# nicochunger/evidence

Hardware: AMD Instinct MI355X
Metric: live_point_logL_evals_per_sec (higher is better)
Workload: dtype f64

## Files before the change

### evidence_amd/csrc/rvll_math.h

```cpp
#pragma once
#include <hip/hip_runtime.h>
#include <stdint.h>

#define RVLL_HD __host__ __device__ __forceinline__

namespace rvll {

RVLL_HD double as_double(uint64_t u) { return __builtin_bit_cast(double, u); }
RVLL_HD uint64_t as_u64(double d) { return __builtin_bit_cast(uint64_t, d); }

struct SincosConsts {
    double S1, S2, S3, S4, S5, S6, C1, C2, C3, C4, C5, C6, TWO_OVER_PI, PIO2_HI, PIO2_LO, MAGIC;
};
RVLL_HD SincosConsts sincos_consts()
{
    return SincosConsts{-1.66666666666666324348e-01, 8.33333333332248946124e-03, -1.98412698298579493134e-04,
                        2.75573137070700676789e-06, -2.50507602534068634195e-08, 1.58969099521155010221e-10,
                        4.16666666666666019037e-02, -1.38888888888741095749e-03, 2.48015872894767294178e-05,
                        -2.75573143513906633035e-07, 2.08757232129817482790e-09, -1.13596475577881948265e-11,
                        6.36619772367581382433e-01, 1.57079632679489655800e+00, 6.12323399573676603587e-17,
                        6755399441055744.0};
}
#if defined(__HIP_DEVICE_COMPILE__)
__device__ __forceinline__ SincosConsts sincos_consts_pinned()
// ... 421 lines not shown
    reduce_dd(x, r, q);
    double sr, cr;
#ifdef RVLL_CR_SERIES_ONLY
    sincos_dd_kernel(r, sr, cr);
#else
    if (__builtin_expect(!sincos_dd_table(r, sr, cr), 0)) sincos_dd_kernel(r, sr, cr);
#endif
    const double s = (q & 1u) ? cr : sr, c = (q & 1u) ? sr : cr;
    const double ss = (q & 2u) ? -s : s, cc = ((q + 1u) & 2u) ? -c : c;
    s_out = x < 0. ? -ss : ss;
    c_out = cc;
}

RVLL_HD double recip_refined(double d)
{
#if defined(__HIP_DEVICE_COMPILE__)
    double y = __builtin_amdgcn_rcp(d);
    double e = __builtin_fma(-d, y, 1.0);
    y = __builtin_fma(y, e, y);
    e = __builtin_fma(-d, y, 1.0);
    return __builtin_fma(y, e, y);
#else
    return 1.0 / d;
#endif
}
RVLL_HD double div_1nr(double n, double d)
{
#if defined(__HIP_DEVICE_COMPILE__)
    double y = __builtin_amdgcn_rcp(d);
    y = __builtin_fma(y, __builtin_fma(-d, y, 1.0), y);
    const double q = n * y;
    return __builtin_fma(__builtin_fma(-d, q, n), y, q);
#else
    return n / d;
#endif
}
RVLL_HD double div_exact(double n, double d) { return div_1nr(n, d); }
RVLL_HD double div_fast(double n, double d) { return div_1nr(n, d); }

RVLL_HD double log_pos(double v)
{
#if defined(__HIP_DEVICE_COMPILE__)
    if (!(v > 0.0 && v < __builtin_inf())) return log(v);
    double m = __builtin_amdgcn_frexp_mant(v);
    int    k = __builtin_amdgcn_frexp_exp(v);
    const bool lowhalf = m < 7.07106781186547524401e-01;
    m = lowhalf ? m + m : m;
    k = lowhalf ? k - 1 : k;
    const double f = m - 1.0;
    const double s = div_fast(f, 2.0 + f);
    const double z = s * s;
    constexpr double L7 = 1.479819860511658591e-01, L6 = 1.531383769920937332e-01, L5 = 1.818357216161805012e-01,
                     L4 = 2.222219843214978396e-01, L3 = 2.857142874366239149e-01, L2 = 3.999999999940941908e-01,
                     L1 = 6.666666666666735130e-01;
    double R;
    asm("v_fma_f64 %0, %1, %2, %3\n\t"
        "v_fma_f64 %0, %1, %0, %4\n\t"
        "v_fma_f64 %0, %1, %0, %5\n\t"
        "v_fma_f64 %0, %1, %0, %6\n\t"
        "v_fma_f64 %0, %1, %0, %7\n\t"
        "v_fma_f64 %0, %1, %0, %8\n\t"
        "v_mul_f64 %0, %0, %1"
        : "=&v"(R)
        : "v"(z), "v"(L7), "v"(L6), "v"(L5), "v"(L4), "v"(L3), "v"(L2), "v"(L1));
    const double hfsq = 0.5 * f * f;
    const double dk = (double)k;
    const double inner = __builtin_fma(s, hfsq + R, dk * 1.90821492927058770002e-10);
    return __builtin_fma(dk, 6.93147180369123816490e-01, -((hfsq - inner) - f));
#else
    return __builtin_log(v);
#endif
}

RVLL_HD void rotate_small(double h, double& s, double& c)
{
    const double h2 = h * h;
    const double sh = h * __builtin_fma(h2, -1.66666666666666666667e-01, 1.0);
    const double ch1 = h2 * __builtin_fma(h2, 4.16666666666666666667e-02, -0.5);
    const double s0 = s, c0 = c;
    s = s0 + __builtin_fma(s0, ch1, c0 * sh);
    c = c0 + __builtin_fma(c0, ch1, -(s0 * sh));
}

RVLL_HD void rotate_mid(double h, double& s, double& c, const SincosConsts& k)
{
    const double S1 = k.S1, S2 = k.S2, S3 = k.S3, S4 = k.S4, S5 = k.S5, S6 = k.S6;
    const double C1 = k.C1, C2 = k.C2, C3 = k.C3, C4 = k.C4, C5 = k.C5, C6 = k.C6;
    double sh, cm1;
#if defined(__HIP_DEVICE_COMPILE__)
    double z, t;
    asm("v_mul_f64 %2, %4, %4\n\t"
        "v_fma_f64 %0, %2, %10, %9\n\t"
        "v_fma_f64 %1, %2, %16, %15\n\t"
        "v_fma_f64 %0, %2, %0, %8\n\t"
        "v_fma_f64 %1, %2, %1, %14\n\t"
        "v_fma_f64 %0, %2, %0, %7\n\t"
        "v_fma_f64 %1, %2, %1, %13\n\t"
        "v_fma_f64 %0, %2, %0, %6\n\t"
        "v_fma_f64 %1, %2, %1, %12\n\t"
        "v_fma_f64 %0, %2, %0, %5\n\t"
        "v_fma_f64 %1, %2, %1, %11\n\t"
        "v_mul_f64 %3, %4, %2\n\t"
        "v_fma_f64 %1, %2, %1, -0.5\n\t"
        "v_fma_f64 %0, %3, %0, %4\n\t"
        "v_mul_f64 %1, %2, %1"
        : "=&v"(sh), "=&v"(cm1), "=&v"(z), "=&v"(t)
        : "v"(h), "s"(S1), "s"(S2), "s"(S3), "s"(S4), "s"(S5), "v"(S6),
          "s"(C1), "s"(C2), "s"(C3), "s"(C4), "s"(C5), "v"(C6));
#else
    const double z = h * h;
    double ps = __builtin_fma(z, S6, S5);
    double pc = __builtin_fma(z, C6, C5);
    ps = __builtin_fma(z, ps, S4);
    pc = __builtin_fma(z, pc, C4);
    ps = __builtin_fma(z, ps, S3);
    pc = __builtin_fma(z, pc, C3);
    ps = __builtin_fma(z, ps, S2);
    pc = __builtin_fma(z, pc, C2);
    ps = __builtin_fma(z, ps, S1);
    pc = __builtin_fma(z, pc, C1);
    const double t = h * z;
    pc = __builtin_fma(z, pc, -0.5);
    sh = __builtin_fma(t, ps, h);
    cm1 = z * pc;
#endif
    const double s0 = s, c0 = c;
    s = __builtin_fma(c0, sh, __builtin_fma(s0, cm1, s0));
    c = __builtin_fma(-s0, sh, __builtin_fma(c0, cm1, c0));
}

RVLL_HD void rotate_mid(double h, double& s, double& c) { rotate_mid(h, s, c, sincos_consts()); }

constexpr double kRotateMidMax = 7.85398163397448279e-01;

template <bool CHECKED>
RVLL_HD void newton_next_sincos(double E, double h, int k, double& s, double& c, const SincosConsts& kc)
{
    if (k == 0) {
        if constexpr (CHECKED) sincos_any(E, s, c, kc);
        else                   sincos_f64(E, s, c, kc);
    } else {
        rotate_mid(h, s, c, kc);
        if (__builtin_expect(!(__builtin_fabs(h) <= kRotateMidMax), 0)) {
            if constexpr (CHECKED) sincos_any(E, s, c, kc);
            else                   sincos_f64(E, s, c, kc);
        }
    }
}

RVLL_HD void quadrant_f32(float sr, float cr, uint32_t uq, float& s_out, float& c_out)
{
    const uint32_t m = 0u - (uq & 1u);
    const uint32_t sb = __builtin_bit_cast(uint32_t, sr), cb = __builtin_bit_cast(uint32_t, cr);
    uint32_t rs, rc;
#if defined(__HIP_DEVICE_COMPILE__)
    asm("v_bfi_b32 %0, %2, %4, %3\n\t"
        "v_bfi_b32 %1, %2, %3, %4"
        : "=&v"(rs), "=&v"(rc) : "v"(m), "v"(sb), "v"(cb));
#else
    rs = (cb & m) | (sb & ~m);
    rc = (sb & m) | (cb & ~m);
#endif
    rs ^= (uq & 2u) << 30;
    rc ^= ((uq + 1u) & 2u) << 30;
    s_out = __builtin_bit_cast(float, rs);
    c_out = __builtin_bit_cast(float, rc);
// ... 94 lines not shown
```

### evidence_amd/csrc/rvll_tile.h

```cpp
#pragma once
#include "rvll_kernels.h"
#include "rvll_math.h"
#include "rvll_special.h"

namespace rvll {

namespace {

constexpr double kTwoPi = 6.283185307179586476925286766559;

__device__ __forceinline__ double slot_get(const rvll_slot s, const double* th)
{
    return s.idx >= 0 ? th[s.idx] : s.val;
}

__device__ __forceinline__ double slot_lds(const rvll_slot* s, const double* th)
{
    const int idx = s->idx;
    const double v = s->val;
    const double tv = th[idx >= 0 ? idx : 0];
    return idx >= 0 ? tv : v;
}

__device__ __forceinline__ double wave_sum(double v)
// ... 123 lines not shown
    const rvll_prior& pr = priors[d];
    const double q = cube_row[d];
    switch (pr.kind) {
    case RVLL_PRIOR_UNIFORM:
        return pr.args[0] + (pr.args[1] - pr.args[0]) * q;
    case RVLL_PRIOR_JEFFREYS:
        return pr.args[0] * pow(pr.args[1] / pr.args[0], q);
    case RVLL_PRIOR_MODJEFFREYS:
        return pr.args[0] * pow(1 + pr.args[1] / pr.args[0], q) - pr.args[0];
    case RVLL_PRIOR_UNIFORMFREQUENCY:
        return pr.args[0] / (1 - q * (pr.args[1] - pr.args[0]) / pr.args[1]);
    case RVLL_PRIOR_NORMAL:
        return (q >= 0. && q <= 1.) ? ndtri_cephes(q) * pr.args[1] + pr.args[0] : NAN;
    case RVLL_PRIOR_LOGNORMAL:
        return (q >= 0. && q <= 1.) ? exp(pr.args[0] * ndtri_cephes(q)) * pr.args[2] + pr.args[1] : NAN;
    case RVLL_PRIOR_TRUNCRAYLEIGH: {
        const double sg = pr.args[0], xm = pr.args[1];
        const double A = 1 - exp(-(xm * xm) / (2 * (sg * sg)));
        return sqrt(-2 * (sg * sg) * log(1 - (q * A))); }
    case RVLL_PRIOR_TABLE:
        return table_ppf(pr, q);
    case RVLL_PRIOR_ALPHA:
        return alpha_ppf(q, pr.args[0], pr.args[1]);
    case RVLL_PRIOR_SORTED_UNIFORM:
    case RVLL_PRIOR_SORTED_LOGUNIFORM:
        return sorted_prior(priors, D, cube_row, d, pr.kind);
    default:
        return NAN;
    }
}

__device__ double prior_heavy(const rvll_prior& pr, double q)
{
    const bool direct = pr.table_post != 0;
    if (pr.kind == RVLL_PRIOR_BETA)
        return beta_ppf_table(q, pr.args[0], pr.args[1], pr.args[2], pr.table_cdf, pr.table_x, direct);
    return gamma_ppf_table(q, pr.args[0], pr.args[1], pr.args[2], pr.table_cdf, pr.table_x, direct);
}

__device__ __forceinline__ double prior_heavy_slim(const rvll_prior& pr, double q, double umax, bool& deferred)
{
    if (pr.table_post != 0 && q > 0. && q < 1.) {
        const double ud = logit_fast(q);
        if (fabs(ud) <= umax) {
            const double z = quintic_table(pr.table_cdf, pr.table_x, ud);
            return pr.kind == RVLL_PRIOR_BETA ? 1. / (1. + exp(-z)) : exp(z) * (1.0 / pr.args[1]);
        }
    }
    deferred = true;
    return NAN;
}

__device__ __forceinline__ double walk_normal(unsigned long long seed, unsigned long long ctr)
{
    const double u1 = uniform01(seed, ctr), u2 = uniform01(seed, ctr + 1);
    double sn, cs;
    sincos_f64(kTwoPi * u2, sn, cs);
    return sqrt(-2. * log_pos(1. - u1)) * cs;
}

struct ItemCtx {
    const double* pp;
    const double* ins;
    const double* dr;
    const double* lin;
    int* nfail;
    int* anyfail;
    int* jfail;
    const int* wide;
    int* pflags;
};

__device__ __forceinline__ bool f32_astray(float E, float Mf, float tolf) { return !(fabsf(E - Mf) <= 1.0f + tolf); }

template <int PREC, bool FAILCHECK, bool EXTRAS = true, bool CR = false, int NP = 0>
__device__ __forceinline__ double eval_item(const LoglikeArgs& a, const ItemCtx& cx, int pl, int j)
{
    const double t  = a.t[j];
    const double y  = a.y[j];
    const double s2 = a.s2[j];
    const int    in = a.inst[j];

    const double2 oj = *reinterpret_cast<const double2*>(cx.ins + (pl * a.Ni + in) * 2);
    double rvm = 0. + oj.x;
    const double var = s2 + oj.y;

    const int Np = NP > 0 ? NP : a.Np;
    if (Np > 0) {
        const bool wide = __builtin_amdgcn_readfirstlane(*cx.wide) != 0;
        bool point_failed = false;
        if constexpr (FAILCHECK) point_failed = cx.anyfail[pl] != 0;
        double ksum = 0.;
#pragma clang loop unroll_count(NP > 0 ? NP : 1)
        for (int ip = 0; ip < Np; ++ip) {
            const double* P = cx.pp + (pl * Np + ip) * kPlanetFields;
            const double2 p01 = *reinterpret_cast<const double2*>(P);
            const double2 p23 = *reinterpret_cast<const double2*>(P + 2);
            const double2 p45 = *reinterpret_cast<const double2*>(P + 4);
            const double  C0  = P[6];
            const double ec = p23.y;
            double rv;
            if (FAILCHECK && point_failed && j >= cx.jfail[pl * Np + ip]) {
                rv = p45.x + C0;
            } else if constexpr (PREC == RVLL_PREC_FP64) {
                const double M = p01.x * (t - p01.y) + p23.x;
                double E = M, s, c, dE = __builtin_inf();
#ifdef RVLL_LOCAL_CONSTS
                const SincosConsts kc = sincos_consts_pinned();
#else
                const SincosConsts kc = sincos_consts();
#endif
                const bool shortcut = a.itmax > kSafeSteps && !wide;
                if (shortcut) {
                    int steps = 0;
                    do {
                        newton_next_sincos<false>(E, dE, steps, s, c, kc);
                        const double f  = E - ec * s - M;
                        const double fp = 1 - ec * c;
                        const double En = E - div_exact(f, fp);
                        dE = En - E;
                        E = En;
                        ++steps;
                    } while (fabs(dE) > a.tol && steps < kSafeSteps);
                }
                if constexpr (CR) {
                    if (!shortcut && a.itmax > kSafeSteps) {
                        int steps = 0;
                        do {
                            newton_next_sincos<true>(E, dE, steps, s, c, kc);
                            const double f  = E - ec * s - M;
                            const double fp = 1 - ec * c;
                            const double En = E - div_exact(f, fp);
                            dE = En - E;
                            E = En;
                            ++steps;
                        } while (fabs(dE) > a.tol && steps < kSafeSteps);
                    }
                }
                bool hit_itmax = false, wander = false;
                if (__builtin_expect(!(fabs(dE) <= a.tol), 0)) {
#ifdef RVLL_AB_PRIO
                    __builtin_amdgcn_s_setprio(2);
#endif
                    int steps = shortcut ? kSafeSteps : 0;
                    if constexpr (CR) { E = M; steps = 0; }
                    do {
#ifdef RVLL_CR_FAKE
                        sincos_any(E, s, c, kc);
#else
                        if constexpr (CR)            sincos_cr(E, s, c);
                        else if (steps < kSafeSteps) newton_next_sincos<true>(E, dE, steps, s, c, kc);
                        else                         sincos_any(E, s, c, kc);
#endif
                        const double f  = E - ec * s - M;
                        const double fp = 1 - ec * c;
                        const double En = E - div_exact(f, fp);
                        dE = En - E;
                        E = En;
                        ++steps;
                    } while (fabs(dE) > a.tol && steps < a.itmax);
                    hit_itmax = steps >= a.itmax;
                    if (steps > kSafeSteps) {
                        atomicOr(&cx.pflags[pl], RVLL_FLAG_WANDERED);
                        if constexpr (!CR) { if (a.cr_redo) { atomicOr(cx.nfail, 2); wander = true; } }
                    }
#ifdef RVLL_AB_PRIO
                    __builtin_amdgcn_s_setprio(0);
#endif
                }
                if (hit_itmax) {
                    if constexpr (CR) {
                        if (atomicMin(&cx.jfail[pl * Np + ip], j) > j) atomicOr(cx.nfail, 4);
                        atomicOr(&cx.anyfail[pl], 1);
                        rv = p45.x + C0;
                    } else {
                        atomicMin(&cx.jfail[pl * Np + ip], j);
                        atomicOr(&cx.anyfail[pl], 1);
                        atomicOr(cx.nfail, 1);
                        rv = p45.x + C0;
                    }
                } else {
                    if (a.tol <= 1e-3) rotate_small(dE, s, c);
                    else               sincos_any(E, s, c, kc);
                    const double den = __builtin_fma(-ec, c, 1.0);
                    const double num = __builtin_fma(p45.x, c - ec, -(p45.y * s));
                    rv = div_fast(num, den) + C0;
                    if constexpr (!CR && !FAILCHECK) { if (__builtin_expect(wander, 0)) rv = __builtin_nan(""); }
                }
            } else {
                const double M = p01.x * (t - p01.y) + p23.x;
                const float Mf = reduce_2pi_to_f32(M);
                const float ecf = (float)ec, tolf = (float)a.tol;
                float E = Mf, s, c, dE;
                int steps = 0;
                do {
                    sincos_f32(E, s, c);
                    const float f  = E - ecf * s - Mf;
                    const float fp = 1.0f - ecf * c;
                    const float En = E - div_f32(f, fp);
                    dE = En - E;
                    E = En;
                    ++steps;
                } while (!(fabsf(dE) <= tolf) && steps < a.itmax && steps < kF32Steps);
                if ((!(fabsf(dE) <= tolf) || f32_astray(E, Mf, tolf)) && steps < a.itmax) {
                    double Ed = M, sd, cd, dd;
                    const SincosConsts kc = sincos_consts();
                    steps = 0;
                    do {
                        sincos_any(Ed, sd, cd, kc);
                        const double f  = Ed - ec * sd - M;
                        const double fp = 1 - ec * cd;
                        const double En = Ed - div_exact(f, fp);
                        dd = En - Ed;
                        Ed = En;
                        ++steps;
                    } while (fabs(dd) > a.tol && steps < a.itmax);
                    if (steps > kSafeSteps) atomicOr(&cx.pflags[pl], RVLL_FLAG_WANDERED);
                    if (steps < a.itmax) {
                        sincos_any(Ed, sd, cd, kc);
                        rv = div_fast(__builtin_fma(p45.x, cd - ec, -(p45.y * sd)), __builtin_fma(-ec, cd, 1.0)) + C0;
                    }
                } else if (steps < a.itmax) {
                    if (steps > kSafeSteps) atomicOr(&cx.pflags[pl], RVLL_FLAG_WANDERED);
                    sincos_f32(E, s, c);
                    const float den = __builtin_fmaf(-ecf, c, 1.0f);
                    const float num = __builtin_fmaf((float)p45.x, c - ecf, -((float)p45.y * s));
                    rv = (double)(div_f32(num, den) + (float)C0);
                }
                if (steps >= a.itmax) {
                    atomicMin(&cx.jfail[pl * Np + ip], j);
                    atomicOr(&cx.anyfail[pl], 1);
                    atomicOr(cx.nfail, 1);
                    rv = p45.x + C0;
                }
            }
            ksum += rv;
        }
        rvm += ksum;
    }

    if constexpr (EXTRAS) {
        if (a.has_drift) {
            const double* d = cx.dr + pl * 6;
            const double tt = (t - d[4]) * (1.0 / 365.25);
            const double t2 = tt * tt;
            rvm += d[0] * tt + d[1] * t2 + d[2] * (t2 * tt) + d[3] * (t2 * t2);
        }
        for (int k = 0; k < a.nlin; ++k)
            rvm += cx.lin[pl * a.nlin + k] * a.linpar[(size_t)k * a.Ne + j];
    }

    const double res = y - rvm;
#ifdef RVLL_AB_NO_LOGDET
    if constexpr (PREC == RVLL_PREC_FP32) {
        const float rf = (float)res, vf = (float)var;
        return (double)(0.5f * __logf(vf) + div_f32(rf * rf, 2.0f * vf));
    } else {
        return 0.5 * log_pos(var) + div_fast(res * res, 2 * var);
    }
#else
    if constexpr (PREC == RVLL_PREC_FP32) {
        const float rf = (float)res, vf = (float)var;
        return (double)div_f32(rf * rf, 2.0f * vf);
    } else {
        return div_fast(res * res, 2 * var);
    }
#endif
}

template <int PREC, bool EXTRAS>
__device__ __forceinline__ double pair_tail(const LoglikeArgs& a, const ItemCtx& cx, int pl, int j, double t, double y, double var, double rvm)
{
    if constexpr (EXTRAS) {
        if (a.has_drift) {
            const double* d = cx.dr + pl * 6;
            const double tt = (t - d[4]) * (1.0 / 365.25);
            const double t2 = tt * tt;
            rvm += d[0] * tt + d[1] * t2 + d[2] * (t2 * tt) + d[3] * (t2 * t2);
        }
        for (int k = 0; k < a.nlin; ++k)
            rvm += cx.lin[pl * a.nlin + k] * a.linpar[(size_t)k * a.Ne + j];
    }
    const double res = y - rvm;
    if constexpr (PREC == RVLL_PREC_FP32) {
        const float rf = (float)res, vf = (float)var;
        return (double)div_f32(rf * rf, 2.0f * vf);
    } else {
        return div_fast(res * res, 2 * var);
    }
}

__device__ __forceinline__ bool pair_solve_f64(const LoglikeArgs& a, const ItemCtx& cx, int pl, double M, double ec, double A, double Bq,
                                               double C0, double& rv)
{
    double Ed = M, sd, cd, dd;
    const SincosConsts kc = sincos_consts();
    int steps = 0;
    do {
        sincos_any(Ed, sd, cd, kc);
        const double f  = Ed - ec * sd - M;
        const double fp = 1 - ec * cd;
        const double En = Ed - div_exact(f, fp);
        dd = En - Ed;
        Ed = En;
        ++steps;
    } while (fabs(dd) > a.tol && steps < a.itmax);
    if (steps > kSafeSteps) atomicOr(&cx.pflags[pl], RVLL_FLAG_WANDERED);
    if (steps >= a.itmax) return false;
    sincos_any(Ed, sd, cd, kc);
    rv = div_fast(__builtin_fma(A, cd - ec, -(Bq * sd)), __builtin_fma(-ec, cd, 1.0)) + C0;
    return true;
}

template <int PREC, bool EXTRAS, int NP = 0>
__device__ __forceinline__ void eval_item_pair(const LoglikeArgs& a, const ItemCtx& cx, int plA, int jA, int plB, int jB,
                                               double& outA, double& outB)
{
    const double tA = a.t[jA], yA = a.y[jA], tB = a.t[jB], yB = a.y[jB];
    const double2 ojA = *reinterpret_cast<const double2*>(cx.ins + (plA * a.Ni + a.inst[jA]) * 2);
    const double2 ojB = *reinterpret_cast<const double2*>(cx.ins + (plB * a.Ni + a.inst[jB]) * 2);
    double rvmA = 0. + ojA.x, rvmB = 0. + ojB.x;
    const double varA = a.s2[jA] + ojA.y, varB = a.s2[jB] + ojB.y;
    const int Np = NP > 0 ? NP : a.Np;
    const f32x2 tolf = splat2((float)a.tol);
    double ksumA = 0., ksumB = 0.;
#pragma clang loop unroll_count(NP > 0 ? NP : 1)
    for (int ip = 0; ip < Np; ++ip) {
        const double* PA = cx.pp + (plA * Np + ip) * kPlanetFields;
        const double* PB = cx.pp + (plB * Np + ip) * kPlanetFields;
        const double2 a01 = *reinterpret_cast<const double2*>(PA), a23 = *reinterpret_cast<const double2*>(PA + 2);
        const double2 b01 = *reinterpret_cast<const double2*>(PB), b23 = *reinterpret_cast<const double2*>(PB + 2);
        const double2 a45 = *reinterpret_cast<const double2*>(PA + 4), b45 = *reinterpret_cast<const double2*>(PB + 4);
        const double aC0 = PA[6], bC0 = PB[6];
        const double MA = a01.x * (tA - a01.y) + a23.x;
// ... 57 lines not shown

#ifndef RVLL_DECODE_INLINE
#define RVLL_DECODE_INLINE __forceinline__
#endif
__device__ __forceinline__ void item_of(int i0, int lane, int Ne, int& pl, int& j)
{
    const int u0 = __builtin_amdgcn_readfirstlane(i0);
    const int pl0 = u0 / Ne;
    pl = pl0;
    j = u0 - pl0 * Ne + lane;
    while (j >= Ne) { j -= Ne; ++pl; }
}

struct TileLds {
    double *theta_s, *pp, *ins, *dr, *lin, *acc, *lay, *contrib;
    int *nfail, *ticket, *wide, *pflags, *anyfail, *jfail;
};
__device__ __forceinline__ TileLds tile_views(const LoglikeArgs& a, double* smem)
{
    const Carve cv = carve(a.PB, a.D, a.Np, a.Ni, a.nlin, a.CH);
    TileLds L;
    L.theta_s = smem + cv.theta;  L.pp = smem + cv.pp;    L.ins = smem + cv.ins;  L.dr = smem + cv.dr;
    L.lin = smem + cv.lin;        L.acc = smem + cv.acc;  L.lay = smem + cv.lay;  L.contrib = smem + cv.contrib;
    int* ints = reinterpret_cast<int*>(smem + cv.ints);
    L.nfail = ints;  L.ticket = ints + 1;  L.wide = ints + 2;  L.pflags = ints + 4;  L.anyfail = L.pflags + a.PB;  L.jfail = L.anyfail + a.PB;
    return L;
}

template <int FUSED, int NT>
__device__ __forceinline__ void tile_stage(const LoglikeArgs& __restrict__ a, const TileLds& L, long long p0, int npts,
                                           unsigned long long* stamp = nullptr, const double* cube_rows = nullptr)
{
    const int tid = threadIdx.x;
    for (int i = tid; i < npts; i += NT) { L.acc[i] = 0.; L.pflags[i] = 0; L.anyfail[i] = 0; }
    for (int i = tid; i < npts * a.Np; i += NT) L.jfail[i] = 0x7fffffff;
    if (tid == 0) { L.nfail[0] = 0; L.ticket[0] = 0; L.wide[0] = 0; }
    if constexpr (FUSED == kFusedSlim) __syncthreads();
    if constexpr (FUSED != kFusedNone) {
        const double* src = cube_rows ? cube_rows : a.cube + p0 * a.D;
        double* dst = (NT != kCuThreads && !cube_rows) ? a.theta_out + p0 * a.D : nullptr;
        const int n_light = a.D - a.n_heavy;
        for (int i = tid; i < npts * n_light; i += NT) {
            const int k = i / npts, pl = i - k * npts;
            const int d = a.light_dims[k];
            const double v = prior_light(a.priors, a.D, src + pl * a.D, d);
            L.theta_s[pl * a.D + d] = v;
            if (dst) dst[pl * a.D + d] = v;
        }
        for (int i = NT - 1 - tid; i < npts * a.n_heavy; i += NT) {
            const int k = i / npts, pl = i - k * npts;
            const int d = a.heavy_dims[k];
            double v;
            if constexpr (FUSED == kFusedSlim) {
                bool deferred = false;
                v = prior_heavy_slim(a.priors[d], src[pl * a.D + d], a.slim_umax, deferred);
                if (deferred) {
                    atomicOr(&L.pflags[pl], kFlagDeferred);
                    if (a.defer) atomicOr(a.defer, 1);
                }
            } else {
                v = prior_heavy(a.priors[d], src[pl * a.D + d]);
            }
            L.theta_s[pl * a.D + d] = v;
            if (dst) dst[pl * a.D + d] = v;
        }
    } else {
        const double* src = cube_rows ? cube_rows : a.theta + p0 * a.D;
        for (int i = tid; i < npts * a.D; i += NT) L.theta_s[i] = src[i];
        if (stamp && tid == 0) {
            __builtin_amdgcn_s_waitcnt(0);
            *stamp = __builtin_amdgcn_s_memrealtime();
        }
    }
    for (int i = tid; i < layout_doubles(a.Np, a.Ni, a.nlin); i += NT) L.lay[i] = a.layblob[i];
}

template <int NT>
__device__ RVLL_DECODE_INLINE void tile_decode(const LoglikeArgs& __restrict__ a, const TileLds& L, int npts)
{
    const int tid = threadIdx.x;
    const rvll_planet* lp = reinterpret_cast<const rvll_planet*>(L.lay);
    const rvll_inst*   li = reinterpret_cast<const rvll_inst*>(L.lay + a.Np * kPlanetDoubles);
    const rvll_slot*   ll = reinterpret_cast<const rvll_slot*>(L.lay + a.Np * kPlanetDoubles + a.Ni * kInstDoubles);
    for (int wk = tid; wk < npts * a.Np; wk += NT) {
        const int pl = wk / a.Np;
        const int k  = wk - pl * a.Np;
        const double* th = L.theta_s + pl * a.D;
        const rvll_planet d = lp[k];
        const double tk = th[max(d.k.idx, 0)], tp = th[max(d.p.idx, 0)], t1 = th[max(d.e1.idx, 0)],
                     t2 = th[max(d.e2.idx, 0)], ta = th[max(d.anom.idx, 0)], te = th[max(d.epoch.idx, 0)];
        const double kraw = d.k.idx >= 0 ? tk : d.k.val;
        const double praw = d.p.idx >= 0 ? tp : d.p.val;
        const double K = d.k_kind == RVLL_K_LOGK1 ? exp(kraw) : kraw;
        const double Pd = d.p_kind == RVLL_P_LOGPERIOD ? exp(praw) : praw;
        const double e1 = d.e1.idx >= 0 ? t1 : d.e1.val;
        const double e2 = d.e2.idx >= 0 ? t2 : d.e2.val;
        double ecc, omega;
        if (d.ecc_kind == RVLL_ECC_SECOS_SESIN) {
            ecc = e1 * e1 + e2 * e2;
            omega = atan2(e2, e1);
            if (ecc > 1) atomicOr(&L.pflags[pl], RVLL_FLAG_INVALID_ORBIT);
        } else if (d.ecc_kind == RVLL_ECC_ECOS_ESIN) {
            ecc = sqrt(e1 * e1 + e2 * e2);
            omega = atan2(e2, e1);
            if (ecc > 1) atomicOr(&L.pflags[pl], RVLL_FLAG_INVALID_ORBIT);
        } else {
            ecc = e1;
            omega = e2;
        }
        const double anom = d.anom.idx >= 0 ? ta : d.anom.val;
        const double ma0 = d.anom_kind == RVLL_ANOM_ML0 ? anom - omega : anom;
        const double ec = ecc > 0.99 ? 0.99 : ecc;
#ifndef RVLL_AB_NO_ROT
        if (ec >= kLongSolveEcc)
            atomicMax(L.ticket, ((int)((ec - kLongSolveEcc) * 340.) << (kTicketBits + kTicketRoundBits)) |
                                (min((pl * a.Ne) >> 6, kTicketRoundMask) << kTicketBits));
#endif
        double so, co;
        sincos_any(omega, so, co);
        const double q = sqrt((1. - ec) * (1. + ec));
        double* P = L.pp + (pl * a.Np + k) * kPlanetFields;
        P[0] = kTwoPi / Pd;
        P[1] = d.epoch.idx >= 0 ? te : d.epoch.val;
        P[2] = ma0;
        P[3] = ec;
        P[4] = K * co;
        P[5] = K * q * so;
        P[6] = K * (ecc * co);
        const double ep = d.epoch.idx >= 0 ? te : d.epoch.val;
        const double mbound = fabs(kTwoPi / Pd) * fmax(fabs(a.tmax - ep), fabs(a.tmin - ep)) + fabs(ma0);
        if (!(mbound < kExcursionM)) atomicOr(L.wide, 1);
        P[7] = 0.;
    }
    for (int pl = NT - 1 - tid; pl < npts; pl += NT) {
        const double* th = L.theta_s + pl * a.D;
        for (int i = 0; i < a.Ni; ++i) {
            L.ins[(pl * a.Ni + i) * 2] = slot_lds(&li[i].offset, th);
            double j2 = 0.;
            if (a.has_jitter) { const double jit = slot_lds(&li[i].jitter, th); j2 = jit * jit; }
            L.ins[(pl * a.Ni + i) * 2 + 1] = j2;
        }
        if (a.has_drift) {
            const rvll_slot* ld = ll + a.nlin;
            double* d = L.dr + pl * 6;
            d[0] = slot_lds(&ld[0], th);
            d[1] = slot_lds(&ld[1], th);
            d[2] = slot_lds(&ld[2], th);
            d[3] = slot_lds(&ld[3], th);
            d[4] = a.tref_from_data ? a.t[0] : slot_lds(&ld[4], th);
            d[5] = 0.;
        }
        for (int k2 = 0; k2 < a.nlin; ++k2) L.lin[pl * a.nlin + k2] = slot_lds(&ll[k2], th);
    }
}

__device__ __forceinline__ int logdet_group(int Ne) { return Ne > 512 ? kWave : 16; }
__device__ __forceinline__ void logdet_finish(const TileLds& L, int pl, int sub, int gs, double m, int e)
{
    double v = __builtin_fma((double)e, 6.93147180559945286227e-01, log_pos(m));
    if (gs == kWave) {
        v = wave_sum_lane0(v);
    } else {
        v += lanes_up_row<8>(v);
        v += lanes_up_row<4>(v);
        v += lanes_up_row<2>(v);
        v += lanes_up_row<1>(v);
    }
    if (sub == 0) L.acc[pl] = 0.5 * v;
}
template <int NT>
__device__ __forceinline__ void tile_logdet(const LoglikeArgs& __restrict__ a, const TileLds& L, int npts)
{
    const int gs = logdet_group(a.Ne);
    const int tid = threadIdx.x, sub = tid & (gs - 1);
    for (int pl = tid / gs; pl < npts; pl += NT / gs) {
        const double* jit = L.ins + pl * a.Ni * 2 + 1;
        double m = 1.;
        int e = 0, since = 0;
#pragma unroll 4
        for (int j = sub; j < a.Ne; j += gs) {
            const double var = a.s2[j] + jit[a.inst[j] * 2];
            m *= __builtin_amdgcn_frexp_mant(var);
            e += __builtin_amdgcn_frexp_exp(var);
            if (++since == 512) {
                e += __builtin_amdgcn_frexp_exp(m);
                m = __builtin_amdgcn_frexp_mant(m);
                since = 0;
            }
        }
        logdet_finish(L, pl, sub, gs, m, e);
    }
}
constexpr int kLogdetPre = 16;
struct LogdetPre {
    double s2[kLogdetPre];
    int inst[kLogdetPre];
    bool valid;
};
__device__ __forceinline__ void logdet_preload(const LoglikeArgs& a, LogdetPre& pre)
{
    const int gs = logdet_group(a.Ne), sub = threadIdx.x & (gs - 1);
    pre.valid = a.Ne <= kLogdetPre * gs;
#pragma unroll
    for (int u = 0; u < kLogdetPre; ++u) {
        const int j = sub + u * gs;
        const bool in = pre.valid && (int)threadIdx.x < gs && j < a.Ne;
        pre.s2[u] = in ? a.s2[j] : 1.;
        pre.inst[u] = in ? a.inst[j] : 0;
    }
}
__device__ __forceinline__ void tile_logdet_pre(const LoglikeArgs& __restrict__ a, const TileLds& L, const LogdetPre& pre)
{
    const int gs = logdet_group(a.Ne), tid = threadIdx.x, sub = tid & (gs - 1);
    if (tid >= gs) return;
    const double* jit = L.ins + 1;
    double m = 1.;
    int e = 0;
#pragma unroll
    for (int u = 0; u < kLogdetPre; ++u)
        if (sub + u * gs < a.Ne) {
// ... 107 lines not shown
                [[maybe_unused]] int r2 = 0;
                if constexpr (PREC != RVLL_PREC_FP64) {
                    if (lane == 0) r = atomicAdd(L.ticket, pairs ? 2 : 1);
                } else {
                    if (lane == 0) r = atomicAdd(L.ticket, 1);
                }
                r = __builtin_amdgcn_readfirstlane(r);
#ifndef RVLL_AB_NO_ROT
                const int r0 = (r >> kTicketBits) & kTicketRoundMask;
                r &= (1 << kTicketBits) - 1;
                if (r * kWave >= cend) break;
                r2 = r + 1;
                r += r0;
                if (r * kWave >= cend) r -= (cend + kWave - 1) >> 6;
#else
                if (r * kWave >= cend) break;
                r2 = r + 1;
#endif
                const int i = r * kWave + lane;
                if constexpr (PREC != RVLL_PREC_FP64) {
                    if (pairs) {
                        const bool has2 = r2 * kWave < cend;
#ifndef RVLL_AB_NO_ROT
                        r2 += r0;
                        if (r2 * kWave >= cend) r2 -= (cend + kWave - 1) >> 6;
#endif
                        if (!has2) r2 = r;
                        const int i2 = r2 * kWave + lane;
                        int plA, jA, plB, jB;
                        item_of(r * kWave, lane, a.Ne, plA, jA);
                        item_of(r2 * kWave, lane, a.Ne, plB, jB);
                        const bool okA = i < cend, okB = has2 && i2 < cend;
                        if (!okA) { plA = 0; jA = 0; }
                        if (!okB) { plB = plA; jB = jA; }
                        double oA, oB;
                        eval_item_pair<PREC, EXTRAS, NP>(a, cx, plA, jA, plB, jB, oA, oB);
                        if (okA) contrib[i] = oA;
                        if (okB) contrib[i2] = oB;
                        continue;
                    }
                }
                if (i < cend) {
                    int pl, j;
                    item_of(r * kWave, lane, a.Ne, pl, j);
                    contrib[i] = eval_item<PREC, false, EXTRAS, false, NP>(a, cx, pl, j);
                }
            }
            if constexpr (TRACE) { if (tid == 0) tr[4] = __builtin_amdgcn_s_memrealtime(); }
        } else {
            bool done = false;
            if constexpr (PREC != RVLL_PREC_FP64) {
                if (pairs) {
                    for (int i = base + tid; i < cend; i += 2 * NT) {
                        const int i2 = i + NT;
                        const bool wave2 = i2 - lane < cend, okB = i2 < cend;
                        int plA, jA, plB, jB;
                        item_of(i - lane, lane, a.Ne, plA, jA);
                        item_of(wave2 ? i2 - lane : i - lane, lane, a.Ne, plB, jB);
                        if (!okB) { plB = plA; jB = jA; }
                        double oA, oB;
                        eval_item_pair<PREC, EXTRAS, NP>(a, cx, plA, jA, plB, jB, oA, oB);
                        contrib[i - base] = oA;
                        if (okB) contrib[i2 - base] = oB;
                    }
                    done = true;
                }
            }
            if (!done)
            for (int i = base + tid; i < cend; i += NT) {
                int pl, j;
                item_of(i - lane, lane, a.Ne, pl, j);
                contrib[i - base] = eval_item<PREC, false, EXTRAS, false, NP>(a, cx, pl, j);
            }
            if constexpr (TRACE) { if (lane == 0) tr[2 + wave] = __builtin_amdgcn_s_memrealtime(); }
        }
        __syncthreads();
        RVLL_TILE_STAMP(2);
        if constexpr (TRACE && DYN) { if (tid == 0) tr[5] = __builtin_amdgcn_s_memrealtime(); }
        if (__builtin_expect(L.nfail[0] != 0, 0)) {
            for (;;) {
                for (int i = base + tid; i < cend; i += NT) {
                    const int pl = i / a.Ne;
                    if (L.anyfail[pl] || contrib[i - base] != contrib[i - base])
                        contrib[i - base] = eval_item<PREC, true, EXTRAS, PREC == RVLL_PREC_FP64, NP>(a, cx, pl, i - pl * a.Ne);
                }
                __syncthreads();
                if (PREC != RVLL_PREC_FP64 || !(L.nfail[0] & 4)) break;
                __syncthreads();
                if (tid == 0) L.nfail[0] &= ~4;
                __syncthreads();
            }
        }
        const int pl_lo = base / a.Ne;
        const int pl_hi = (cend - 1) / a.Ne;
        const int nslices = (a.Ne + kTileWindow - 1) / kTileWindow;
        for (int pl0 = pl_lo + wave; pl0 <= pl_hi; pl0 += 4 * NW) {
            for (int sl = 0; sl < nslices; ++sl) {
                int lo[4], hi[4];
                double v[4];
#pragma unroll
                for (int k = 0; k < 4; ++k) {
                    const int pl = pl0 + k * NW;
                    const int first = pl * a.Ne + sl * kTileWindow;
                    const int l = max(base, first), h = min(min(cend, (pl + 1) * a.Ne), first + kTileWindow);
                    const bool any = pl <= pl_hi && l < h;
                    lo[k] = any ? l : 0;
                    hi[k] = any ? h : 0;
                }
                point_partials4(contrib, base, lo, hi, lane, v);
                if (lane == 0) {
#pragma unroll
                    for (int k = 0; k < 4; ++k) if (lo[k] < hi[k]) L.acc[pl0 + k * NW] += v[k];
                }
            }
        }
        __syncthreads();
    }

    for (int pl = tid; pl < npts; pl += NT) tile_write_point(a, L, p0, pl);
    RVLL_TILE_STAMP(3);
#undef RVLL_TILE_STAMP
    if constexpr (TRACE) {
        __syncthreads();
        if (threadIdx.x == 0) tr[6] = __builtin_amdgcn_s_memrealtime();
    }
}


}

}
```

Baseline: 270.3 million.

## Pool per-planet RV fractions into one division and precompute constant offset sum

In the FP64 path, each planet's velocity term num/den is no longer divided separately. The terms are combined as a running fraction (N, D) and one division is done at the end inside the chi-square computation. The per-planet constant C0 terms are pre-summed into P[7] during the per-point setup, which is restructured so each wave handles several points' planets per lane. The fail-recheck path also picks the CR variant only when itmax exceeds the safe step count. Together these remove one division per planet per item, at some risk of overflow or precision loss from multiplying denominators, and they change the setup's work mapping.

```diff
diff --git a/evidence_amd/csrc/rvll_math.h b/evidence_amd/csrc/rvll_math.h
--- a/evidence_amd/csrc/rvll_math.h
+++ b/evidence_amd/csrc/rvll_math.h
@@ -527,6 +527,25 @@
     c = c0 + __builtin_fma(c0, ch1, -(s0 * sh));
 }
 
+struct ItemPool {
+    double N, D;
+};
+RVLL_HD void pool_add(ItemPool& p, bool first, double num, double den)
+{
+    if (first) {
+        p.N = num;
+        p.D = den;
+    } else {
+        p.N = __builtin_fma(num, p.D, p.N * den);
+        p.D = p.D * den;
+    }
+}
+RVLL_HD double pool_chi2(const ItemPool& p, double R, double var)
+{
+    const double T = __builtin_fma(R, p.D, -p.N);
+    return div_fast(T * T, (var + var) * (p.D * p.D));
+}
+
 RVLL_HD void rotate_mid(double h, double& s, double& c, const SincosConsts& k)
 {
     const double S1 = k.S1, S2 = k.S2, S3 = k.S3, S4 = k.S4, S5 = k.S5, S6 = k.S6;
diff --git a/evidence_amd/csrc/rvll_tile.h b/evidence_amd/csrc/rvll_tile.h
--- a/evidence_amd/csrc/rvll_tile.h
+++ b/evidence_amd/csrc/rvll_tile.h
@@ -229,26 +229,29 @@
     const int    in = a.inst[j];
 
     const double2 oj = *reinterpret_cast<const double2*>(cx.ins + (pl * a.Ni + in) * 2);
-    double rvm = 0. + oj.x;
+    double rvm = PREC == RVLL_PREC_FP64 ? oj.x : 0. + oj.x;
     const double var = s2 + oj.y;
 
     const int Np = NP > 0 ? NP : a.Np;
+    [[maybe_unused]] ItemPool pool{0., 1.};
     if (Np > 0) {
         const bool wide = __builtin_amdgcn_readfirstlane(*cx.wide) != 0;
         bool point_failed = false;
         if constexpr (FAILCHECK) point_failed = cx.anyfail[pl] != 0;
         double ksum = 0.;
+        if constexpr (PREC == RVLL_PREC_FP64) rvm += cx.pp[pl * Np * kPlanetFields + 7];
 #pragma clang loop unroll_count(NP > 0 ? NP : 1)
         for (int ip = 0; ip < Np; ++ip) {
             const double* P = cx.pp + (pl * Np + ip) * kPlanetFields;
             const double2 p01 = *reinterpret_cast<const double2*>(P);
             const double2 p23 = *reinterpret_cast<const double2*>(P + 2);
             const double2 p45 = *reinterpret_cast<const double2*>(P + 4);
-            const double  C0  = P[6];
             const double ec = p23.y;
-            double rv;
+            [[maybe_unused]] double num, den;
+            [[maybe_unused]] double rv;
             if (FAILCHECK && point_failed && j >= cx.jfail[pl * Np + ip]) {
-                rv = p45.x + C0;
+                if constexpr (PREC == RVLL_PREC_FP64) { num = p45.x; den = 1.0; }
+                else                                  rv = p45.x + P[6];
             } else if constexpr (PREC == RVLL_PREC_FP64) {
                 const double M = p01.x * (t - p01.y) + p23.x;
                 double E = M, s, c, dE = __builtin_inf();
@@ -319,22 +322,22 @@
                     if constexpr (CR) {
                         if (atomicMin(&cx.jfail[pl * Np + ip], j) > j) atomicOr(cx.nfail, 4);
                         atomicOr(&cx.anyfail[pl], 1);
-                        rv = p45.x + C0;
                     } else {
                         atomicMin(&cx.jfail[pl * Np + ip], j);
                         atomicOr(&cx.anyfail[pl], 1);
                         atomicOr(cx.nfail, 1);
-                        rv = p45.x + C0;
                     }
+                    num = p45.x;
+                    den = 1.0;
                 } else {
                     if (a.tol <= 1e-3) rotate_small(dE, s, c);
                     else               sincos_any(E, s, c, kc);
-                    const double den = __builtin_fma(-ec, c, 1.0);
-                    const double num = __builtin_fma(p45.x, c - ec, -(p45.y * s));
-                    rv = div_fast(num, den) + C0;
-                    if constexpr (!CR && !FAILCHECK) { if (__builtin_expect(wander, 0)) rv = __builtin_nan(""); }
+                    den = __builtin_fma(-ec, c, 1.0);
+                    num = __builtin_fma(p45.x, c - ec, -(p45.y * s));
+                    if constexpr (!CR && !FAILCHECK) { if (__builtin_expect(wander, 0)) num = __builtin_nan(""); }
                 }
             } else {
+                const double C0 = P[6];
                 const double M = p01.x * (t - p01.y) + p23.x;
                 const float Mf = reduce_2pi_to_f32(M);
                 const float ecf = (float)ec, tolf = (float)a.tol;
@@ -381,9 +384,10 @@
                     rv = p45.x + C0;
                 }
             }
-            ksum += rv;
-        }
-        rvm += ksum;
+            if constexpr (PREC == RVLL_PREC_FP64) pool_add(pool, ip == 0, num, den);
+            else                                  ksum += rv;
+        }
+        if constexpr (PREC != RVLL_PREC_FP64) rvm += ksum;
     }
 
     if constexpr (EXTRAS) {
@@ -397,6 +401,13 @@
             rvm += cx.lin[pl * a.nlin + k] * a.linpar[(size_t)k * a.Ne + j];
     }
 
+    if constexpr (PREC == RVLL_PREC_FP64) {
+#ifdef RVLL_AB_NO_LOGDET
+        return 0.5 * log_pos(var) + pool_chi2(pool, y - rvm, var);
+#else
+        return pool_chi2(pool, y - rvm, var);
+#endif
+    }
     const double res = y - rvm;
 #ifdef RVLL_AB_NO_LOGDET
     if constexpr (PREC == RVLL_PREC_FP32) {
@@ -620,60 +631,79 @@
     const rvll_planet* lp = reinterpret_cast<const rvll_planet*>(L.lay);
     const rvll_inst*   li = reinterpret_cast<const rvll_inst*>(L.lay + a.Np * kPlanetDoubles);
     const rvll_slot*   ll = reinterpret_cast<const rvll_slot*>(L.lay + a.Np * kPlanetDoubles + a.Ni * kInstDoubles);
-    for (int wk = tid; wk < npts * a.Np; wk += NT) {
-        const int pl = wk / a.Np;
-        const int k  = wk - pl * a.Np;
-        const double* th = L.theta_s + pl * a.D;
-        const rvll_planet d = lp[k];
-        const double tk = th[max(d.k.idx, 0)], tp = th[max(d.p.idx, 0)], t1 = th[max(d.e1.idx, 0)],
-                     t2 = th[max(d.e2.idx, 0)], ta = th[max(d.anom.idx, 0)], te = th[max(d.epoch.idx, 0)];
-        const double kraw = d.k.idx >= 0 ? tk : d.k.val;
-        const double praw = d.p.idx >= 0 ? tp : d.p.val;
-        const double K = d.k_kind == RVLL_K_LOGK1 ? exp(kraw) : kraw;
-        const double Pd = d.p_kind == RVLL_P_LOGPERIOD ? exp(praw) : praw;
-        const double e1 = d.e1.idx >= 0 ? t1 : d.e1.val;
-        const double e2 = d.e2.idx >= 0 ? t2 : d.e2.val;
-        double ecc, omega;
-        if (d.ecc_kind == RVLL_ECC_SECOS_SESIN) {
-            ecc = e1 * e1 + e2 * e2;
-            omega = atan2(e2, e1);
-            if (ecc > 1) atomicOr(&L.pflags[pl], RVLL_FLAG_INVALID_ORBIT);
-        } else if (d.ecc_kind == RVLL_ECC_ECOS_ESIN) {
-            ecc = sqrt(e1 * e1 + e2 * e2);
-            omega = atan2(e2, e1);
-            if (ecc > 1) atomicOr(&L.pflags[pl], RVLL_FLAG_INVALID_ORBIT);
-        } else {
-            ecc = e1;
-            omega = e2;
-        }
-        const double anom = d.anom.idx >= 0 ? ta : d.anom.val;
-        const double ma0 = d.anom_kind == RVLL_ANOM_ML0 ? anom - omega : anom;
-        const double ec = ecc > 0.99 ? 0.99 : ecc;
+    const int lane_d = tid & (kWave - 1);
+    const int ppw = a.Np <= kWave ? kWave / max(a.Np, 1) : 1;
+    const int nchunk = a.Np <= kWave ? 1 : (a.Np + kWave - 1) / kWave;
+    const int q_d = a.Np <= kWave ? lane_d / max(a.Np, 1) : 0;
+    const int k_d = lane_d - q_d * a.Np;
+    for (int g = tid >> 6, c = 0; g * ppw < npts && a.Np > 0; ) {
+        const int pl = g * ppw + q_d;
+        const int k = k_d + c * kWave;
+        const bool mine = q_d < ppw && pl < npts;
+        if (mine && k < a.Np) {
+            const double* th = L.theta_s + pl * a.D;
+            const rvll_planet d = lp[k];
+            const double tk = th[max(d.k.idx, 0)], tp = th[max(d.p.idx, 0)], t1 = th[max(d.e1.idx, 0)],
+                         t2 = th[max(d.e2.idx, 0)], ta = th[max(d.anom.idx, 0)], te = th[max(d.epoch.idx, 0)];
+            const double kraw = d.k.idx >= 0 ? tk : d.k.val;
+            const double praw = d.p.idx >= 0 ? tp : d.p.val;
+            const double K = d.k_kind == RVLL_K_LOGK1 ? exp(kraw) : kraw;
+            const double Pd = d.p_kind == RVLL_P_LOGPERIOD ? exp(praw) : praw;
+            const double e1 = d.e1.idx >= 0 ? t1 : d.e1.val;
+            const double e2 = d.e2.idx >= 0 ? t2 : d.e2.val;
+            double ecc, omega;
+            if (d.ecc_kind == RVLL_ECC_SECOS_SESIN) {
+                ecc = e1 * e1 + e2 * e2;
+                omega = atan2(e2, e1);
+                if (ecc > 1) atomicOr(&L.pflags[pl], RVLL_FLAG_INVALID_ORBIT);
+            } else if (d.ecc_kind == RVLL_ECC_ECOS_ESIN) {
+                ecc = sqrt(e1 * e1 + e2 * e2);
+                omega = atan2(e2, e1);
+                if (ecc > 1) atomicOr(&L.pflags[pl], RVLL_FLAG_INVALID_ORBIT);
+            } else {
+                ecc = e1;
+                omega = e2;
+            }
+            const double anom = d.anom.idx >= 0 ? ta : d.anom.val;
+            const double ma0 = d.anom_kind == RVLL_ANOM_ML0 ? anom - omega : anom;
+            const double ec = ecc > 0.99 ? 0.99 : ecc;
 #ifndef RVLL_AB_NO_ROT
-        if (ec >= kLongSolveEcc)
-            atomicMax(L.ticket, ((int)((ec - kLongSolveEcc) * 340.) << (kTicketBits + kTicketRoundBits)) |
-                                (min((pl * a.Ne) >> 6, kTicketRoundMask) << kTicketBits));
-#endif
-        double so, co;
-        sincos_any(omega, so, co);
-        const double q = sqrt((1. - ec) * (1. + ec));
-        double* P = L.pp + (pl * a.Np + k) * kPlanetFields;
-        P[0] = kTwoPi / Pd;
-        P[1] = d.epoch.idx >= 0 ? te : d.epoch.val;
-        P[2] = ma0;
-        P[3] = ec;
-        P[4] = K * co;
-        P[5] = K * q * so;
-        P[6] = K * (ecc * co);
-        const double ep = d.epoch.idx >= 0 ? te : d.epoch.val;
-        const double mbound = fabs(kTwoPi / Pd) * fmax(fabs(a.tmax - ep), fabs(a.tmin - ep)) + fabs(ma0);
-        if (!(mbound < kExcursionM)) atomicOr(L.wide, 1);
-        P[7] = 0.;
+            if (ec >= kLongSolveEcc)
+                atomicMax(L.ticket, ((int)((ec - kLongSolveEcc) * 340.) << (kTicketBits + kTicketRoundBits)) |
+                                    (min((pl * a.Ne) >> 6, kTicketRoundMask) << kTicketBits));
+#endif
+            double so, co;
+            sincos_any(omega, so, co);
+            const double q = sqrt((1. - ec) * (1. + ec));
+            double* P = L.pp + (pl * a.Np + k) * kPlanetFields;
+            P[0] = kTwoPi / Pd;
+            P[1] = d.epoch.idx >= 0 ? te : d.epoch.val;
+            P[2] = ma0;
+            P[3] = ec;
+            P[4] = K * co;
+            P[5] = K * q * so;
+            P[6] = K * (ecc * co);
+            const double ep = d.epoch.idx >= 0 ? te : d.epoch.val;
+            const double mbound = fabs(kTwoPi / Pd) * fmax(fabs(a.tmax - ep), fabs(a.tmin - ep)) + fabs(ma0);
+            if (!(mbound < kExcursionM)) atomicOr(L.wide, 1);
+            P[7] = 0.;
+        }
+        __builtin_amdgcn_fence(__ATOMIC_RELEASE, "wavefront");
+        __builtin_amdgcn_wave_barrier();
+        __builtin_amdgcn_fence(__ATOMIC_ACQUIRE, "wavefront");
+        const bool last = c == nchunk - 1;
+        if (last && mine && k_d == 0) {
+            double* P0 = L.pp + pl * a.Np * kPlanetFields;
+            double sum = P0[6];
+            for (int k2 = 1; k2 < a.Np; ++k2) sum += P0[k2 * kPlanetFields + 6];
+            P0[7] = sum;
+        }
+        if (last) { c = 0; g += NT / kWave; } else ++c;
     }
     for (int pl = NT - 1 - tid; pl < npts; pl += NT) {
         const double* th = L.theta_s + pl * a.D;
         for (int i = 0; i < a.Ni; ++i) {
-            L.ins[(pl * a.Ni + i) * 2] = slot_lds(&li[i].offset, th);
+            L.ins[(pl * a.Ni + i) * 2] = 0. + slot_lds(&li[i].offset, th);
             double j2 = 0.;
             if (a.has_jitter) { const double jit = slot_lds(&li[i].jitter, th); j2 = jit * jit; }
             L.ins[(pl * a.Ni + i) * 2 + 1] = j2;
@@ -947,7 +977,8 @@
                 for (int i = base + tid; i < cend; i += NT) {
                     const int pl = i / a.Ne;
                     if (L.anyfail[pl] || contrib[i - base] != contrib[i - base])
-                        contrib[i - base] = eval_item<PREC, true, EXTRAS, PREC == RVLL_PREC_FP64, NP>(a, cx, pl, i - pl * a.Ne);
+                        contrib[i - base] = a.itmax > kSafeSteps ? eval_item<PREC, true, EXTRAS, PREC == RVLL_PREC_FP64, NP>(a, cx, pl, i - pl * a.Ne)
+                                                                 : eval_item<PREC, true, EXTRAS, false, NP>(a, cx, pl, i - pl * a.Ne);
                 }
                 __syncthreads();
                 if (PREC != RVLL_PREC_FP64 || !(L.nfail[0] & 4)) break;
```

Measured after the change: 277.8 million (median of 6 runs). 1.03x the previous value.
